# pierremtb/PINNs-TF2.0

Measured on NVIDIA B200. Metric: collocation-points/sec per training step (1D Burgers 8x20 tanh, Adam step), higher is better.
Workload: dtype f64

## Files before the change

pinns-tf2.0_b200/csrc/burgers_fused_v2.cuh:

```cuda
#pragma once
#include "burgers_fused.cuh"

namespace pinn {
namespace burgers2 {

using burgers::W;
using burgers::NHID;
using burgers::P_NET;
using burgers::WPAD;
using burgers::TILE;
using burgers::PSTRIDE;
using burgers::IDX_DL1;
using burgers::IDX_DL2;
using burgers::IDX_LD;
using burgers::IDX_LF;
using burgers::woff;
using burgers::boff;
using burgers::prow;
using burgers::Args;

constexpr int CHAINS = 4;
constexpr int THREADS = 256;
constexpr int ROUND = CHAINS * TILE;
#ifndef PINN_RING
#define PINN_RING 2
#endif
#ifndef PINN_ABL_NOWG
#define PINN_ABL_NOWG 0
#endif
#ifndef PINN_ABL_NOACT
#define PINN_ABL_NOACT 0
#endif
#ifndef PINN_ABL_NODMMA
#define PINN_ABL_NODMMA 0
#endif
constexpr int RING = PINN_RING;

constexpr int STASH0 = 640;
constexpr int STASHL = 640;
constexpr int STASH_PER_WARP = STASH0 + 6 * STASHL;
constexpr int SM_W = 0;
constexpr int SM_STASH = SM_W + WPAD;
constexpr int SM_RING = SM_STASH + CHAINS * STASH_PER_WARP;
constexpr int RED_PER_WARP = 128;
constexpr int SM_RED = SM_RING + CHAINS * RING * 640;
constexpr int SM_BAR = SM_RED + CHAINS * RED_PER_WARP;
constexpr int SM_SPECIAL = SM_BAR + 1 + 2 * CHAINS * RING + 1;
constexpr int SM_DOUBLES = SM_SPECIAL + 32 * W;
constexpr int SMEM_BYTES = SM_DOUBLES * 8;

__device__ __forceinline__ void mbar_arrive(uint64_t* bar) {
  asm volatile("mbarrier.arrive.shared::cta.b64 _, [%0];" ::"r"(smem_u32(bar)) : "memory");
}
__device__ __forceinline__ uint64_t* bar_full(uint64_t* bars, int c, int slot) { return bars + 1 + (c * RING + slot) * 2; }
__device__ __forceinline__ uint64_t* bar_empty(uint64_t* bars, int c, int slot) { return bars + 2 + (c * RING + slot) * 2; }
__device__ __forceinline__ void wait_produced(uint64_t* bars, int c, int T) { mbar_wait(bar_full(bars, c, T % RING), (T / RING) & 1); }
__device__ __forceinline__ void wait_consumed(uint64_t* bars, int c, int T) { mbar_wait(bar_empty(bars, c, T % RING), (T / RING) & 1); }

__device__ __forceinline__ int unit5(int j, int q) { return j < 4 ? 8 * (j >> 1) + 2 * q + (j & 1) : (q < 2 ? 16 + 2 * q : 13 + 2 * q); }

__device__ __forceinline__ void c_to_v5(double (&V)[4][5], const double (&Z)[4][3][2], int lane) {
#pragma unroll
  for (int s = 0; s < 4; s++) {
    V[s][0] = Z[s][0][0]; V[s][1] = Z[s][0][1]; V[s][2] = Z[s][1][0]; V[s][3] = Z[s][1][1];
    const double odd = __shfl_sync(0xffffffffu, Z[s][2][1], (lane & ~3) | (lane & 1));
    V[s][4] = (lane & 2) ? odd : Z[s][2][0];
  }
}

__device__ __forceinline__ void mma_layer5(double (&Z)[4][3][2], const double (&V)[4][5], const double* Wl, int ldk, int ldn,
                                           int lane) {
  const int g = lane >> 2, q = lane & 3;
#pragma unroll
  for (int ks = 0; ks < 5; ks++) {
    const int k = unit5(ks, q);
    double b[3];
#pragma unroll
    for (int nt = 0; nt < 3; nt++) {
      const int n = 8 * nt + g;
      b[nt] = (n < W) ? Wl[k * ldk + n * ldn] : 0.0;
    }
#pragma unroll
    for (int s = 0; s < 4; s++)
#pragma unroll
      for (int nt = 0; nt < 3; nt++) dmma(Z[s][nt], V[s][ks], b[nt]);
  }
}

__device__ __forceinline__ void act_forward5(double (&V)[4][5]) {
  if (PINN_ABL_NOACT) return;
#pragma unroll
  for (int j = 0; j < 5; j++) {
    const double a = tanh_fast(V[0][j]);
    const double zx = V[1][j];
    const double s = fma(-a, a, 1.0);
    V[0][j] = a;
    V[1][j] = s * zx;
    V[2][j] = s * V[2][j];
    V[3][j] = s * fma(-2.0 * a * zx, zx, V[3][j]);
  }
}

__device__ __forceinline__ void act_backward5(double (&A)[4][5], const double (&H)[4][5]) {
  if (PINN_ABL_NOACT) return;
#pragma unroll
  for (int j = 0; j < 5; j++) {
    const double a = H[0][j], ax = H[1][j], at = H[2][j], axx = H[3][j];
    const double A0 = A[0][j], Ax = A[1][j], At = A[2][j], Axx = A[3][j];
    const double s = fma(-a, a, 1.0);
    const double u1 = fma(ax, Ax, at * At);
    const double u2 = fma(a, axx, ax * ax);
    double z = fma(-2.0 * a, u1, s * A0);
    z = fma(-2.0 * Axx, u2, z);
    A[0][j] = z;
    A[1][j] = fma(-4.0 * a * ax, Axx, s * Ax);
    A[2][j] = s * At;
    A[3][j] = s * Axx;
  }
}

__device__ __forceinline__ void stage5(double* T, const double (&V)[4][5], int lane) {
  const int pg = prow(lane >> 2), q = lane & 3;
  const int u4 = unit5(4, q);
#pragma unroll
  for (int s = 0; s < 4; s++) {
    double* row = T + (8 * s + pg) * W;
    *reinterpret_cast<double2*>(row + 2 * q) = make_double2(V[s][0], V[s][1]);
    *reinterpret_cast<double2*>(row + 8 + 2 * q) = make_double2(V[s][2], V[s][3]);
    row[u4] = V[s][4];
  }
}
__device__ __forceinline__ void load5(double (&V)[4][5], const double* T, int lane) {
  const int pg = prow(lane >> 2), q = lane & 3;
  const int u4 = unit5(4, q);
#pragma unroll
  for (int s = 0; s < 4; s++) {
    const double* row = T + (8 * s + pg) * W;
    const double2 c0 = *reinterpret_cast<const double2*>(row + 2 * q);
    const double2 c1 = *reinterpret_cast<const double2*>(row + 8 + 2 * q);
    V[s][0] = c0.x; V[s][1] = c0.y; V[s][2] = c1.x; V[s][3] = c1.y;
    V[s][4] = row[u4];
  }
}

struct Own { int mt, mask; };
__device__ __forceinline__ Own ownership(int l, int wg) {
  const int k = (wg - l) & 3;
  Own o;
  if (k < 3) { o.mt = k; o.mask = (wg == 3 && l <= 3) ? 3 : 7; }
  else if (l <= 3) { o.mt = (3 - l) & 3; o.mask = 4; }
  else { o.mt = 0; o.mask = 0; }
  return o;
}

template <int L, int MASK>
__device__ __forceinline__ void wgrad_task(double (&acc)[3][2], int mt, const double* Aop, const double* ZB, const double* sm,
                                           double sc0, double sc1, int lane) {
  const int g = lane >> 2, q = lane & 3;
  const double* SP = sm + SM_SPECIAL;
  const double* Wsm = sm + SM_W;
  const int i = 8 * mt + g;
  const double* bp0 = ZB + g + q * W;
  const double* bp1 = ZB + 8 + g + q * W;
  const double* bp2 = (16 + g < W ? ZB + 16 + g : SP + 1) + q * W;
  const double* ap = (i < W ? Aop + i : (i == W ? SP : SP + 1)) + q * W;
#pragma unroll
  for (int ks = 0; ks < 8; ks++) {
    const int st = ks >> 1;
    const int off = (8 * st + 4 * (ks & 1)) * W;
    const double a = ap[off];
    if (MASK & 1) dmma(acc[0], a, bp0[off]);
    if (MASK & 2) dmma(acc[1], a, bp1[off]);
    if (MASK & 4) dmma(acc[2], a, bp2[off]);
  }
}

template <int L>
__device__ __forceinline__ void wgrad_layer(double (&acc)[3][2], int wg, int it, int half, int cnt, const double* sm,
                                            uint64_t* bars, double sc0, double sc1, int lane) {
  constexpr int J = 7 - L;
  const int T = 7 * it + J;
  const int slot = T % RING;
  const Own o = ownership(L, wg);
#pragma unroll 1
  for (int c = 2 * half; c < 2 * half + 2; c++) {
    if (4 * it + c >= cnt) break;
    wait_produced(bars, c, T);
    const double* stash = sm + SM_STASH + c * STASH_PER_WARP;
    const double* Aop = stash + (L - 1) * STASHL;
    const double* ZB = sm + SM_RING + (c * RING + slot) * 640;
    if (!PINN_ABL_NOWG) {
      if (o.mask == 7) wgrad_task<L, 7>(acc, o.mt, Aop, ZB, sm, sc0, sc1, lane);
      else if (o.mask == 3) wgrad_task<L, 3>(acc, o.mt, Aop, ZB, sm, sc0, sc1, lane);
      else if (o.mask == 4) wgrad_task<L, 4>(acc, o.mt, Aop, ZB, sm, sc0, sc1, lane);
    }
    __syncwarp();
    if (lane == 0) mbar_arrive(bar_empty(bars, c, slot));
  }
}

template <int L>
__device__ __forceinline__ void wgrad_flush(const double (&acc)[3][2], int wg, double* outp, int lane) {
  const int g = lane >> 2, q = lane & 3;
  const Own o = ownership(L, wg);
  const int in_dim = W;
  const int i = 8 * o.mt + g;
#pragma unroll
  for (int nt = 0; nt < 3; nt++)
#pragma unroll
    for (int e = 0; e < 2; e++) {
      const int j = 8 * nt + 2 * q + e;
      if (j < W && ((o.mask >> nt) & 1)) {
        if (i < in_dim) outp[woff(L) + i * W + j] = acc[nt][e];
        else if (i == in_dim) outp[boff(L) + j] = acc[nt][e];
      }
    }
}

__global__ void __launch_bounds__(THREADS, 1) fused_loss_grad(const Args p) {
  extern __shared__ __align__(16) double sm[];
  pdl_launch_dependents();
  if (p.run_flag && *p.run_flag != 0) return;
  double* Wsm = sm + SM_W;
  uint64_t* bars = reinterpret_cast<uint64_t*>(sm + SM_BAR);
  const int lane = threadIdx.x & 31, warp = threadIdx.x >> 5;
  const int g = lane >> 2, q = lane & 3;

  for (int i = threadIdx.x; i < 32 * W; i += THREADS) sm[SM_SPECIAL + i] = (i % W == 0 && i / W < 8) ? 1.0 : 0.0;
  if (threadIdx.x == 0) {
    mbar_init(bars, 1);
    for (int i = 0; i < CHAINS * RING; i++) {
      mbar_init(bars + 1 + 2 * i, 1);
      mbar_init(bars + 2 + 2 * i, 4);
    }
  }
  __syncthreads();
  if (threadIdx.x == 0) {
    mbar_expect_tx(bars, WPAD * 8);
    tma_bulk_g2s(Wsm, p.w, WPAD * 8, bars);
  }
  mbar_wait(bars, 0);

  const double sc0 = 2.0 / p.dx0, sc1 = 2.0 / p.dx1;
  const long long tiles_total = (p.n_total + TILE - 1) / TILE;
  const long long tbase = tiles_total / gridDim.x, trem = tiles_total - tbase * gridDim.x;
  const int cnt = (int)(tbase + (blockIdx.x < trem ? 1 : 0));
  const long long first_tile = tbase * blockIdx.x + (blockIdx.x < trem ? blockIdx.x : trem);
  const int my_rounds = (cnt + CHAINS - 1) / CHAINS;
  double* outp = p.partials + (size_t)blockIdx.x * PSTRIDE;

  if (warp >= CHAINS) {
    const int wg = warp & 3;
    double a1[3][2], a2[3][2], a3[3][2], a4[3][2], a5[3][2], a6[3][2], a7[3][2];
#pragma unroll
    for (int s = 0; s < 3; s++)
#pragma unroll
      for (int e = 0; e < 2; e++)
        a1[s][e] = a2[s][e] = a3[s][e] = a4[s][e] = a5[s][e] = a6[s][e] = a7[s][e] = 0.0;
#pragma unroll 1
    for (int it2 = 0; it2 < 2 * my_rounds; it2++) {
      const int it = it2 >> 1, half = it2 & 1;
      wgrad_layer<7>(a7, wg, it, half, cnt, sm, bars, sc0, sc1, lane);
      wgrad_layer<6>(a6, wg, it, half, cnt, sm, bars, sc0, sc1, lane);
      wgrad_layer<5>(a5, wg, it, half, cnt, sm, bars, sc0, sc1, lane);
      wgrad_layer<4>(a4, wg, it, half, cnt, sm, bars, sc0, sc1, lane);
      wgrad_layer<3>(a3, wg, it, half, cnt, sm, bars, sc0, sc1, lane);
      wgrad_layer<2>(a2, wg, it, half, cnt, sm, bars, sc0, sc1, lane);
      wgrad_layer<1>(a1, wg, it, half, cnt, sm, bars, sc0, sc1, lane);
    }
    wgrad_flush<1>(a1, wg, outp, lane);
    wgrad_flush<2>(a2, wg, outp, lane);
    wgrad_flush<3>(a3, wg, outp, lane);
    wgrad_flush<4>(a4, wg, outp, lane);
    wgrad_flush<5>(a5, wg, outp, lane);
    wgrad_flush<6>(a6, wg, outp, lane);
    wgrad_flush<7>(a7, wg, outp, lane);
  } else {
    const int c = warp;
    const int n_tiles = cnt > c ? (cnt - c + CHAINS - 1) / CHAINS : 0;
    double* stash = sm + SM_STASH + c * STASH_PER_WARP;
    const double l1 = p.ide ? Wsm[P_NET] : 1.0;
    const double kap = p.ide ? exp(Wsm[P_NET + 1]) : p.nu;
    double loss_d = 0.0, loss_f = 0.0, gl1 = 0.0, gl2 = 0.0;
    double g8[5], gb8 = 0.0;
    double g0x[5], g0t[5], g0b[5];
#pragma unroll
    for (int j = 0; j < 5; j++) g8[j] = g0x[j] = g0t[j] = g0b[j] = 0.0;
    const int pg = prow(g);
    int u5[5];
#pragma unroll
    for (int j = 0; j < 5; j++) u5[j] = unit5(j, q);
    auto load_xt = [&](int it, double& xo, double& to) {
      long long pt = (first_tile + 4 * it + c) * TILE + g;
      if (pt >= p.n_total) pt = p.n_total - 1;
      if (p.xc && pt >= p.c0 && pt < p.c0 + p.n_c) {
        xo = __ldg(p.xc + (pt - p.c0)); to = __ldg(p.tc + (pt - p.c0));
      } else {
        xo = __ldg(p.x + pt); to = __ldg(p.t + pt);
      }
    };
    double xr_next = 0.0, tr_next = 0.0;
    if (n_tiles > 0) load_xt(0, xr_next, tr_next);

#pragma unroll 1
    for (int it = 0; it < n_tiles; it++) {
      const long long pt = (first_tile + 4 * it + c) * TILE + g;
      const bool in_set = pt < p.n_total;
      const double xr = xr_next, tr = tr_next;
      if (it + 1 < n_tiles) load_xt(it + 1, xr_next, tr_next);
      const double wf = (in_set && pt >= p.c0 && pt < p.c0 + p.n_c) ? p.wf : 0.0;
      const bool has_d = in_set && pt >= p.d0 && pt < p.d0 + p.n_d;
      const double wd = has_d ? p.wd : 0.0;
      const double ut = has_d ? __ldg(p.utgt + (pt - p.d0)) : 0.0;
      const double xh = 2.0 * (xr - p.lb0) / p.dx0 - 1.0;
      const double th = 2.0 * (tr - p.lb1) / p.dx1 - 1.0;

      double V[4][5];
#pragma unroll
      for (int j = 0; j < 5; j++) {
        const double w0 = Wsm[u5[j]], w1 = Wsm[W + u5[j]], b = Wsm[2 * W + u5[j]];
        V[0][j] = fma(xh, w0, fma(th, w1, b));
        V[1][j] = sc0 * w0;
        V[2][j] = sc1 * w1;
        V[3][j] = 0.0;
      }
      act_forward5(V);
      if (it > 0) wait_consumed(bars, c, 7 * (it - 1) + 6);
      stage5(stash, V, lane);
#pragma unroll 1
      for (int l = 1; l < NHID; l++) {
        const double* Wl = Wsm + woff(l);
        double Z[4][3][2];
#pragma unroll
        for (int nt = 0; nt < 3; nt++)
#pragma unroll
          for (int e = 0; e < 2; e++) {
            const int col = 8 * nt + 2 * q + e;
            Z[0][nt][e] = (col < W) ? Wl[W * W + col] : 0.0;
            Z[1][nt][e] = Z[2][nt][e] = Z[3][nt][e] = 0.0;
          }
        if (!PINN_ABL_NODMMA) mma_layer5(Z, V, Wl, W, 1, lane);
        c_to_v5(V, Z, lane);
        act_forward5(V);
        if (l < NHID - 1) stage5(stash + STASH0 + (l - 1) * STASHL, V, lane);
      }
      double A[4][5];
      {
        const double* W8 = Wsm + woff(8);
        double w8[5];
#pragma unroll
        for (int j = 0; j < 5; j++) w8[j] = W8[u5[j]];
        double out[4];
#pragma unroll
        for (int s = 0; s < 4; s++) {
          double acc = 0.0;
#pragma unroll
          for (int j = 0; j < 5; j++) acc = fma(V[s][j], w8[j], acc);
          acc += shfl_xor_d(acc, 1);
          acc += shfl_xor_d(acc, 2);
          out[s] = acc;
        }
        out[0] += Wsm[boff(8)];
        const double u = out[0], ux = out[1], utt = out[2], uxx = out[3];
        const double f = utt + l1 * u * ux - kap * uxx;
        const double r = u - ut;
        const double cc = 2.0 * wf * f;
        double seed[4];
        seed[0] = fma(cc * l1, ux, 2.0 * wd * r);
        seed[1] = cc * l1 * u;
        seed[2] = cc;
        seed[3] = -cc * kap;
        if (q == 0) {
          loss_d = fma(wd * r, r, loss_d);
          loss_f = fma(wf * f, f, loss_f);
          gl1 = fma(cc * u, ux, gl1);
          gl2 = fma(-cc * kap, uxx, gl2);
          gb8 += seed[0];
        }
#pragma unroll
        for (int j = 0; j < 5; j++) {
          double acc = g8[j];
#pragma unroll
          for (int s = 0; s < 4; s++) {
            acc = fma(V[s][j], seed[s], acc);
            A[s][j] = seed[s] * w8[j];
          }
          g8[j] = acc;
        }
      }
#pragma unroll 1
      for (int l = NHID - 1; l >= 1; l--) {
        const int T = 7 * it + (7 - l), slot = T % RING;
        if (l < NHID - 1) load5(V, stash + STASH0 + (l - 1) * STASHL, lane);
        act_backward5(A, V);
        if (T >= RING) wait_consumed(bars, c, T - RING);
        stage5(sm + SM_RING + (c * RING + slot) * 640, A, lane);
        __syncwarp();
        if (lane == 0) mbar_arrive(bar_full(bars, c, slot));
        {
          const double* Wl = Wsm + woff(l);
          double An[4][3][2];
#pragma unroll
          for (int s = 0; s < 4; s++)
#pragma unroll
            for (int nt = 0; nt < 3; nt++) An[s][nt][0] = An[s][nt][1] = 0.0;
          if (!PINN_ABL_NODMMA) mma_layer5(An, A, Wl, 1, W, lane);
          c_to_v5(A, An, lane);
        }
      }
      {
        load5(V, stash, lane);
        act_backward5(A, V);
#pragma unroll
        for (int j = 0; j < 5; j++) {
          g0x[j] = fma(xh, A[0][j], fma(sc0, A[1][j], g0x[j]));
          g0t[j] = fma(th, A[0][j], fma(sc1, A[2][j], g0t[j]));
          g0b[j] += A[0][j];
        }
      }
    }

    double* red = sm + SM_RED + c * RED_PER_WARP;
    loss_d = warp_sum(loss_d); loss_f = warp_sum(loss_f); gl1 = warp_sum(gl1); gl2 = warp_sum(gl2); gb8 = warp_sum(gb8);
#pragma unroll
    for (int j = 0; j < 5; j++) {
      double v = g8[j], vx = g0x[j], vt = g0t[j], vb = g0b[j];
      v += shfl_xor_d(v, 4); v += shfl_xor_d(v, 8); v += shfl_xor_d(v, 16);
      vx += shfl_xor_d(vx, 4); vx += shfl_xor_d(vx, 8); vx += shfl_xor_d(vx, 16);
      vt += shfl_xor_d(vt, 4); vt += shfl_xor_d(vt, 8); vt += shfl_xor_d(vt, 16);
      vb += shfl_xor_d(vb, 4); vb += shfl_xor_d(vb, 8); vb += shfl_xor_d(vb, 16);
      if (g == 0) { red[8 + u5[j]] = v; red[32 + u5[j]] = vx; red[32 + W + u5[j]] = vt; red[32 + 2 * W + u5[j]] = vb; }
    }
    if (lane == 0) { red[0] = loss_d; red[1] = loss_f; red[2] = gl1; red[3] = gl2; red[4] = gb8; }
  }

  __syncthreads();
  {
    const double* red = sm + SM_RED;
    constexpr int R = RED_PER_WARP;
    const int t = threadIdx.x;
    auto sum4 = [&](int i) { return red[i] + red[R + i] + red[2 * R + i] + red[3 * R + i]; };
    if (t < W) outp[woff(8) + t] = sum4(8 + t);
    if (t >= 64 && t < 64 + 3 * W) outp[woff(0) + (t - 64)] = sum4(32 + (t - 64));
    if (t == 32) outp[boff(8)] = sum4(4);
    if (t == 33) outp[IDX_LD] = sum4(0);
    if (t == 34) outp[IDX_LF] = sum4(1);
    if (t == 35) outp[IDX_DL1] = sum4(2);
    if (t == 36) outp[IDX_DL2] = sum4(3);
    if (t == 37) outp[3023] = 0.0;
  }
  if (p.tail.enabled) fused_tail(p.tail, p.partials, PSTRIDE, sm + SM_STASH);
}

}
}
```

Measured before the change: 259.7 million.

## Interleave per-stream DMMA with tanh activation math across layers in fused Burgers kernel

Splits the per-layer forward and backward work into per-stream pieces so DMMA tensor-core ops for the derivative streams and the next layer's value stream run interleaved with FP64 activation math, instead of one long DMMA block followed by one long FP64 block. The backward pass computes each stream's activation adjoint, stages it, and immediately issues its DMMA, with the stash load for the next layer moved after the barrier arrive. The aim is to overlap the tensor-core and FP64 pipes and shorten the serial dependency chain. It raises register pressure (launch bounds swapped for maxnreg 252) and adds a SASS analysis script.

```diff
diff --git a/pinns-tf2.0_b200/csrc/burgers_fused_v2.cuh b/pinns-tf2.0_b200/csrc/burgers_fused_v2.cuh
--- a/pinns-tf2.0_b200/csrc/burgers_fused_v2.cuh
+++ b/pinns-tf2.0_b200/csrc/burgers_fused_v2.cuh
@@ -59,76 +59,80 @@
 
 __device__ __forceinline__ int unit5(int j, int q) { return j < 4 ? 8 * (j >> 1) + 2 * q + (j & 1) : (q < 2 ? 16 + 2 * q : 13 + 2 * q); }
 
-__device__ __forceinline__ void c_to_v5(double (&V)[4][5], const double (&Z)[4][3][2], int lane) {
-#pragma unroll
-  for (int s = 0; s < 4; s++) {
-    V[s][0] = Z[s][0][0]; V[s][1] = Z[s][0][1]; V[s][2] = Z[s][1][0]; V[s][3] = Z[s][1][1];
-    const double odd = __shfl_sync(0xffffffffu, Z[s][2][1], (lane & ~3) | (lane & 1));
-    V[s][4] = (lane & 2) ? odd : Z[s][2][0];
-  }
-}
-
-__device__ __forceinline__ void mma_layer5(double (&Z)[4][3][2], const double (&V)[4][5], const double* Wl, int ldk, int ldn,
-                                           int lane) {
+__device__ __forceinline__ void c_to_v5(double (&v)[5], const double (&Z)[3][2], int lane) {
+  v[0] = Z[0][0]; v[1] = Z[0][1]; v[2] = Z[1][0]; v[3] = Z[1][1];
+  const double odd = __shfl_sync(0xffffffffu, Z[2][1], (lane & ~3) | (lane & 1));
+  v[4] = (lane & 2) ? odd : Z[2][0];
+}
+
+__device__ __forceinline__ void mma_stream5(double (&Z)[3][2], const double (&v)[5], const double* Wl, int ldk, int ldn, int lane) {
+  if (PINN_ABL_NODMMA) return;
   const int g = lane >> 2, q = lane & 3;
 #pragma unroll
   for (int ks = 0; ks < 5; ks++) {
     const int k = unit5(ks, q);
-    double b[3];
 #pragma unroll
     for (int nt = 0; nt < 3; nt++) {
       const int n = 8 * nt + g;
-      b[nt] = (n < W) ? Wl[k * ldk + n * ldn] : 0.0;
-    }
-#pragma unroll
-    for (int s = 0; s < 4; s++)
-#pragma unroll
-      for (int nt = 0; nt < 3; nt++) dmma(Z[s][nt], V[s][ks], b[nt]);
-  }
-}
+      dmma(Z[nt], v[ks], (n < W) ? Wl[k * ldk + n * ldn] : 0.0);
+    }
+  }
+}
+
+template <int S>
+__device__ __forceinline__ double act_forward(double a, double zx, double z) {
+  if (PINN_ABL_NOACT) return z;
+  const double s = fma(-a, a, 1.0);
+  return S == 3 ? s * fma(-2.0 * a * zx, zx, z) : s * z;
+}
+__device__ __forceinline__ double act_value(double z) { return PINN_ABL_NOACT ? z : tanh_fast(z); }
 
 __device__ __forceinline__ void act_forward5(double (&V)[4][5]) {
-  if (PINN_ABL_NOACT) return;
 #pragma unroll
   for (int j = 0; j < 5; j++) {
-    const double a = tanh_fast(V[0][j]);
+    const double a = act_value(V[0][j]);
     const double zx = V[1][j];
-    const double s = fma(-a, a, 1.0);
     V[0][j] = a;
-    V[1][j] = s * zx;
-    V[2][j] = s * V[2][j];
-    V[3][j] = s * fma(-2.0 * a * zx, zx, V[3][j]);
-  }
-}
-
-__device__ __forceinline__ void act_backward5(double (&A)[4][5], const double (&H)[4][5]) {
-  if (PINN_ABL_NOACT) return;
+    V[1][j] = act_forward<1>(a, zx, zx);
+    V[2][j] = act_forward<2>(a, zx, V[2][j]);
+    V[3][j] = act_forward<3>(a, zx, V[3][j]);
+  }
+}
+
+template <int S>
+__device__ __forceinline__ void zbar5(double (&Zb)[5], const double (&A)[4][5], const double (&H)[4][5]) {
 #pragma unroll
   for (int j = 0; j < 5; j++) {
+    if (PINN_ABL_NOACT) { Zb[j] = A[S][j]; continue; }
     const double a = H[0][j], ax = H[1][j], at = H[2][j], axx = H[3][j];
     const double A0 = A[0][j], Ax = A[1][j], At = A[2][j], Axx = A[3][j];
     const double s = fma(-a, a, 1.0);
-    const double u1 = fma(ax, Ax, at * At);
-    const double u2 = fma(a, axx, ax * ax);
-    double z = fma(-2.0 * a, u1, s * A0);
-    z = fma(-2.0 * Axx, u2, z);
-    A[0][j] = z;
-    A[1][j] = fma(-4.0 * a * ax, Axx, s * Ax);
-    A[2][j] = s * At;
-    A[3][j] = s * Axx;
-  }
-}
-
+    if (S == 0) {
+      const double u1 = fma(ax, Ax, at * At);
+      const double u2 = fma(a, axx, ax * ax);
+      double z = fma(-2.0 * a, u1, s * A0);
+      z = fma(-2.0 * Axx, u2, z);
+      Zb[j] = z;
+    } else if (S == 1) {
+      Zb[j] = fma(-4.0 * a * ax, Axx, s * Ax);
+    } else if (S == 2) {
+      Zb[j] = s * At;
+    } else {
+      Zb[j] = s * Axx;
+    }
+  }
+}
+
+__device__ __forceinline__ void stage5(double* T, int s, const double (&v)[5], int lane) {
+  const int pg = prow(lane >> 2), q = lane & 3;
+  double* row = T + (8 * s + pg) * W;
+  *reinterpret_cast<double2*>(row + 2 * q) = make_double2(v[0], v[1]);
+  *reinterpret_cast<double2*>(row + 8 + 2 * q) = make_double2(v[2], v[3]);
+  row[unit5(4, q)] = v[4];
+}
 __device__ __forceinline__ void stage5(double* T, const double (&V)[4][5], int lane) {
-  const int pg = prow(lane >> 2), q = lane & 3;
-  const int u4 = unit5(4, q);
-#pragma unroll
-  for (int s = 0; s < 4; s++) {
-    double* row = T + (8 * s + pg) * W;
-    *reinterpret_cast<double2*>(row + 2 * q) = make_double2(V[s][0], V[s][1]);
-    *reinterpret_cast<double2*>(row + 8 + 2 * q) = make_double2(V[s][2], V[s][3]);
-    row[u4] = V[s][4];
-  }
+#pragma unroll
+  for (int s = 0; s < 4; s++) stage5(T, s, V[s], lane);
 }
 __device__ __forceinline__ void load5(double (&V)[4][5], const double* T, int lane) {
   const int pg = prow(lane >> 2), q = lane & 3;
@@ -217,7 +221,55 @@
     }
 }
 
-__global__ void __launch_bounds__(THREADS, 1) fused_loss_grad(const Args p) {
+__device__ __forceinline__ void bias_init(double (&Z)[3][2], const double* Wl, int q) {
+#pragma unroll
+  for (int nt = 0; nt < 3; nt++)
+#pragma unroll
+    for (int e = 0; e < 2; e++) {
+      const int col = 8 * nt + 2 * q + e;
+      Z[nt][e] = (col < W) ? Wl[W * W + col] : 0.0;
+    }
+}
+
+template <bool LAST>
+__device__ __forceinline__ void forward_layer(double (&V)[4][5], double (&Z0)[3][2], const double* Wsm, int l, double* stash,
+                                              int lane) {
+  const double* Wl = Wsm + woff(l);
+  double a[5];
+  c_to_v5(a, Z0, lane);
+#pragma unroll
+  for (int j = 0; j < 5; j++) a[j] = act_value(a[j]);
+  double Z[3][3][2];
+#pragma unroll
+  for (int s = 0; s < 3; s++)
+#pragma unroll
+    for (int nt = 0; nt < 3; nt++) Z[s][nt][0] = Z[s][nt][1] = 0.0;
+#pragma unroll
+  for (int s = 0; s < 3; s++) mma_stream5(Z[s], V[s + 1], Wl, W, 1, lane);
+  if (!LAST) {
+    bias_init(Z0, Wsm + woff(l + 1), lane & 3);
+    mma_stream5(Z0, a, Wsm + woff(l + 1), W, 1, lane);
+  }
+  double* T = stash + STASH0 + (l - 1) * STASHL;
+#pragma unroll
+  for (int j = 0; j < 5; j++) V[0][j] = a[j];
+  if (!LAST) stage5(T, 0, V[0], lane);
+  double zx[5];
+  c_to_v5(zx, Z[0], lane);
+  c_to_v5(V[2], Z[1], lane);
+  c_to_v5(V[3], Z[2], lane);
+#pragma unroll
+  for (int j = 0; j < 5; j++) {
+    V[1][j] = act_forward<1>(a[j], zx[j], zx[j]);
+    V[2][j] = act_forward<2>(a[j], zx[j], V[2][j]);
+    V[3][j] = act_forward<3>(a[j], zx[j], V[3][j]);
+  }
+  if (!LAST)
+#pragma unroll
+    for (int s = 1; s < 4; s++) stage5(T, s, V[s], lane);
+}
+
+__global__ void __maxnreg__(252) fused_loss_grad(const Args p) {
   extern __shared__ __align__(16) double sm[];
   pdl_launch_dependents();
   if (p.run_flag && *p.run_flag != 0) return;
@@ -325,26 +377,15 @@
         V[3][j] = 0.0;
       }
       act_forward5(V);
+      double Z0[3][2];
+      bias_init(Z0, Wsm + woff(1), q);
+      mma_stream5(Z0, V[0], Wsm + woff(1), W, 1, lane);
       if (it > 0) wait_consumed(bars, c, 7 * (it - 1) + 6);
       stage5(stash, V, lane);
 #pragma unroll 1
-      for (int l = 1; l < NHID; l++) {
-        const double* Wl = Wsm + woff(l);
-        double Z[4][3][2];
-#pragma unroll
-        for (int nt = 0; nt < 3; nt++)
-#pragma unroll
-          for (int e = 0; e < 2; e++) {
-            const int col = 8 * nt + 2 * q + e;
-            Z[0][nt][e] = (col < W) ? Wl[W * W + col] : 0.0;
-            Z[1][nt][e] = Z[2][nt][e] = Z[3][nt][e] = 0.0;
-          }
-        if (!PINN_ABL_NODMMA) mma_layer5(Z, V, Wl, W, 1, lane);
-        c_to_v5(V, Z, lane);
-        act_forward5(V);
-        if (l < NHID - 1) stage5(stash + STASH0 + (l - 1) * STASHL, V, lane);
-      }
-      double A[4][5];
+      for (int l = 1; l < NHID - 1; l++) forward_layer<false>(V, Z0, Wsm, l, stash, lane);
+      forward_layer<true>(V, Z0, Wsm, NHID - 1, stash, lane);
+      double An[4][3][2];
       {
         const double* W8 = Wsm + woff(8);
         double w8[5];
@@ -381,41 +422,72 @@
         for (int j = 0; j < 5; j++) {
           double acc = g8[j];
 #pragma unroll
-          for (int s = 0; s < 4; s++) {
-            acc = fma(V[s][j], seed[s], acc);
-            A[s][j] = seed[s] * w8[j];
-          }
+          for (int s = 0; s < 4; s++) acc = fma(V[s][j], seed[s], acc);
           g8[j] = acc;
         }
+#pragma unroll
+        for (int nt = 0; nt < 3; nt++)
+#pragma unroll
+          for (int e = 0; e < 2; e++) {
+            const int col = 8 * nt + 2 * q + e;
+            const double w = (col < W) ? W8[col] : 0.0;
+#pragma unroll
+            for (int s = 0; s < 4; s++) An[s][nt][e] = seed[s] * w;
+          }
       }
+      double H[4][5];
+#pragma unroll
+      for (int s = 0; s < 4; s++)
+#pragma unroll
+        for (int j = 0; j < 5; j++) H[s][j] = V[s][j];
 #pragma unroll 1
       for (int l = NHID - 1; l >= 1; l--) {
         const int T = 7 * it + (7 - l), slot = T % RING;
-        if (l < NHID - 1) load5(V, stash + STASH0 + (l - 1) * STASHL, lane);
-        act_backward5(A, V);
+        const double* Wl = Wsm + woff(l);
+        double* ring = sm + SM_RING + (c * RING + slot) * 640;
+        double A[4][5], Zb[5];
+        double Bn[4][3][2];
+#pragma unroll
+        for (int s = 0; s < 4; s++)
+#pragma unroll
+          for (int nt = 0; nt < 3; nt++) Bn[s][nt][0] = Bn[s][nt][1] = 0.0;
         if (T >= RING) wait_consumed(bars, c, T - RING);
-        stage5(sm + SM_RING + (c * RING + slot) * 640, A, lane);
+        c_to_v5(A[3], An[3], lane);
+        zbar5<3>(Zb, A, H);
+        stage5(ring, 3, Zb, lane);
+        mma_stream5(Bn[3], Zb, Wl, 1, W, lane);
+        c_to_v5(A[2], An[2], lane);
+        zbar5<2>(Zb, A, H);
+        stage5(ring, 2, Zb, lane);
+        mma_stream5(Bn[2], Zb, Wl, 1, W, lane);
+        c_to_v5(A[1], An[1], lane);
+        zbar5<1>(Zb, A, H);
+        stage5(ring, 1, Zb, lane);
+        mma_stream5(Bn[1], Zb, Wl, 1, W, lane);
+        c_to_v5(A[0], An[0], lane);
+        zbar5<0>(Zb, A, H);
+        stage5(ring, 0, Zb, lane);
         __syncwarp();
         if (lane == 0) mbar_arrive(bar_full(bars, c, slot));
-        {
-          const double* Wl = Wsm + woff(l);
-          double An[4][3][2];
-#pragma unroll
-          for (int s = 0; s < 4; s++)
-#pragma unroll
-            for (int nt = 0; nt < 3; nt++) An[s][nt][0] = An[s][nt][1] = 0.0;
-          if (!PINN_ABL_NODMMA) mma_layer5(An, A, Wl, 1, W, lane);
-          c_to_v5(A, An, lane);
-        }
+        load5(H, stash + (l - 1) * STASHL, lane);
+        mma_stream5(Bn[0], Zb, Wl, 1, W, lane);
+#pragma unroll
+        for (int s = 0; s < 4; s++)
+#pragma unroll
+          for (int nt = 0; nt < 3; nt++) An[s][nt][0] = Bn[s][nt][0], An[s][nt][1] = Bn[s][nt][1];
       }
       {
-        load5(V, stash, lane);
-        act_backward5(A, V);
+        double A[4][5], Z1[5], Z2[5], Z0b[5];
+#pragma unroll
+        for (int s = 0; s < 4; s++) c_to_v5(A[s], An[s], lane);
+        zbar5<0>(Z0b, A, H);
+        zbar5<1>(Z1, A, H);
+        zbar5<2>(Z2, A, H);
 #pragma unroll
         for (int j = 0; j < 5; j++) {
-          g0x[j] = fma(xh, A[0][j], fma(sc0, A[1][j], g0x[j]));
-          g0t[j] = fma(th, A[0][j], fma(sc1, A[2][j], g0t[j]));
-          g0b[j] += A[0][j];
+          g0x[j] = fma(xh, Z0b[j], fma(sc0, Z1[j], g0x[j]));
+          g0t[j] = fma(th, Z0b[j], fma(sc1, Z2[j], g0t[j]));
+          g0b[j] += Z0b[j];
         }
       }
     }
diff --git a/profiles/sass_chain_runs.py b/profiles/sass_chain_runs.py
--- /dev/null
+++ b/profiles/sass_chain_runs.py
@@ -0,0 +1,62 @@
+import os
+import re
+import subprocess
+import sys
+
+ROOT = os.path.dirname(os.path.dirname(os.path.abspath(__file__)))
+LIB = sys.argv[1] if len(sys.argv) > 1 else os.path.join(ROOT, "pinns-tf2.0_b200", "lib", "libpinn_b200.so")
+KERNEL = "_ZN4pinn8burgers215fused_loss_gradENS_7burgers4ArgsE"
+FP64 = {"DFMA", "DMUL", "DADD", "DSETP", "DMNMX", "DSET"}
+
+sass = subprocess.run(["cuobjdump", "-sass", LIB], capture_output=True, text=True, check=True).stdout
+ins, cur = [], None
+for line in sass.splitlines():
+    m = re.search(r"Function : (\S+)", line)
+    if m:
+        cur = m.group(1)
+        continue
+    if cur != KERNEL:
+        continue
+    m = re.match(r"\s*/\*([0-9a-f]{4,})\*/\s+(@!?U?P\w+\s+)?([A-Z][A-Z0-9_]*)(\.[A-Za-z0-9_.]+)?\s*([^;]*);", line)
+    if m:
+        ins.append((int(m.group(1), 16), m.group(3), m.group(5), bool(m.group(2))))
+if not ins:
+    sys.exit("%s: no SASS for %s" % (LIB, KERNEL))
+
+
+def cls(op):
+    return "D" if op == "DMMA" else ("F" if op in FP64 else "o")
+
+
+loops = []
+for addr, op, args, pred in ins:
+    m = re.search(r"0x([0-9a-f]+)", args) if op == "BRA" and pred else None
+    if m and int(m.group(1), 16) <= addr:
+        loops.append((int(m.group(1), 16), addr))
+body = lambda lo, hi: [(a, op) for a, op, _, _ in ins if lo <= a <= hi]
+hot = []
+for lo, hi in loops:
+    ops = [op for _, op in body(lo, hi)]
+    if ops.count("DMMA") >= 15 and any(o in FP64 for o in ops):
+        hot.append((lo, hi))
+inner = [(lo, hi) for lo, hi in hot if not any((l2, h2) != (lo, hi) and lo <= l2 and h2 <= hi for l2, h2 in hot)]
+
+print("# `burgers2::fused_loss_grad` chain-warp layer loops (`cuobjdump -sass %s`)\n" % os.path.relpath(LIB, ROOT))
+for lo, hi in sorted(inner):
+    seq = [cls(op) for _, op in body(lo, hi)]
+    runs = []
+    for c in seq:
+        if runs and runs[-1][0] == c:
+            runs[-1][1] += 1
+        else:
+            runs.append([c, 1])
+    longest, f = 0, 0
+    for c in seq:
+        if c == "D":
+            f = 0
+        elif c == "F":
+            f += 1
+            longest = max(longest, f)
+    print("loop 0x%04x..0x%04x: %d instructions, DMMA %d, FP64 %d, other %d; longest FP64 stretch without a DMMA: %d"
+          % (lo, hi, len(seq), seq.count("D"), seq.count("F"), seq.count("o"), longest))
+    print("  " + " ".join("%s%d" % (c, n) for c, n in runs) + "\n")
```

Result: slower. 244.5 million, median of 6 (-5.9%).
